# fulcrumgenomics/fgumi

Measured on AMD Instinct MI355X. Metric: simplex consensus throughput, input raw reads/s (depth-8 x 150bp), higher is better.
Workload: dtype f64

## Files before the change

### fgumi_amd/csrc/api.cpp

```cpp
#include <chrono>
#include <cstdio>
#include <stdexcept>
#include <cstring>
#include <mutex>
#include <map>
#include <mutex>
#include <string>
#include <thread>
#include "engine.h"
#include <gnu/libc-version.h>
#include <cmath>
#include "fastpath.h"
#include "host_common.h"
#include "simgen.h"
#include "canon_core.h"
#include "reject_core.h"
#include "aln_tags_core.h"

namespace fgx {
using canon::CANON_KIND_DUPLEX; using canon::CANON_KIND_CODEC; using canon::CANON_KIND_SIMPLEX;
uint32_t launch_canon_molecules(hipStream_t s, int kind, const canon::Params& P, const canon::CodecParams& PC, const uint8_t* d_blob,
                                const uint64_t* d_rec_off, const uint32_t* d_rec_len, const uint32_t* d_grp_first, const uint32_t* d_def, uint32_t nd,
                                const uint64_t* d_first, uint8_t* d_out, const uint64_t* d_out_off, uint32_t* d_out_len, int* d_status,
                                canon::Delta* d_delta, DevBuf& slabs, canon::RefRuns* d_runs, const rej::Params* PS);
// ... 1360 lines not shown
  out4[1] = out4[0] - s2_tile_bytes(mean_records);
  out4[2] = (uint32_t)sizeof(FullItem);
  out4[3] = S2_FLAG_DESC_BYTES;
}
void fgx_debug_last_packed_rows(const fgx_caller* c, uint64_t* out2) {
  if (!out2) return;
  out2[0] = out2[1] = 0;
  if (c && c->fast) { out2[0] = c->fast->fp.last_packed_clean; out2[1] = c->fast->fp.last_packed_general; }
}
void fgx_debug_last_full_results(const fgx_caller* c, uint64_t* out4) {
  if (!out4) return;
  for (int i = 0; i < 4; i++) out4[i] = (c && c->fast) ? c->fast->fp.last_full_results[i] : 0;
}
uint64_t fgx_debug_last_full_results_over(const fgx_caller* c) { return (c && c->fast) ? c->fast->fp.last_full_results[4] : 0; }
int fgx_debug_full_range_whole(uint32_t base, uint32_t items, uint32_t cap) { return full_range_whole(base, items, cap) ? 1 : 0; }
void fgx_debug_last_chain(const fgx_caller* c, uint32_t* out2) { if (out2) { out2[0] = (c && c->fast) ? c->fast->fp.last_launches : 0u; out2[1] = (c && c->fast) ? c->fast->fp.last_host_syncs : 0u; } }
uint32_t fgx_debug_last_routed(const fgx_caller* c) { return (c && c->fast) ? c->fast->fp.last_routed : 0u; }
int fgx_debug_last_direct(const fgx_caller* c) { return (c && c->fast) ? c->fast->fp.last_direct : 0; }
void fgx_set_general_only(fgx_caller* c, int on) { if (c) c->general_only = on != 0; }
void fgx_set_fast_lds_bytes(fgx_caller* c, uint32_t bytes) { if (c) { if (!c->fast) c->fast = new FastState(); c->fast->fp.lds_tile_bytes_large = bytes; } }

int fgx_call_columns(fgx_caller* c, const uint8_t* bases, const uint8_t* quals, uint32_t n_cols, uint32_t depth, uint8_t* out_base,
                     uint8_t* out_qual, uint32_t* out_depth, uint32_t* out_errors) {
  if (!c) return 1;
  c->err.clear();
  try {
    ColumnBatch& B = c->batch;
    B.clear();
    std::vector<uint8_t> rb, rq;
    for (uint32_t j0 = 0; j0 < n_cols; j0 += 4096) {
// ... 137 lines not shown
```

### fgumi_amd/csrc/fastpath.h

```cpp
#pragma once
#include <algorithm>
#include "engine.h"

#if defined(__HIPCC__)
#define FP_HD __host__ __device__ __forceinline__
#else
#define FP_HD inline
#endif

namespace fgx {

constexpr int FAST_RX_CAP = 48;

struct EndDesc {
  uint64_t col_off;
  uint64_t first_off;
  uint64_t kept_off;
  uint32_t cons_len;
  uint32_t rec_size;
  uint16_t mi_off, cb_off;
  uint8_t mi_len, cb_len, rx_len, type;
  uint8_t has_cb, has_rx, valid, meth;
  char rx[FAST_RX_CAP];
};
// ... 41 lines not shown
  return mean_need > floor16 ? std::min<uint32_t>((mean_need + 15u) & ~15u, 17408u) : floor16;
}
constexpr uint32_t FULL_ITEM_OBS = 0x80000000u;
constexpr uint32_t FULL_ITEM_CONT = 0x40000000u;

struct FullResult {
  uint32_t w0;
  uint32_t w1;
};
static_assert(sizeof(FullResult) == 8, "a result is one 8-byte store");
constexpr uint32_t FULL_RESULT_NONE = 0xFFu;
constexpr uint32_t FULL_RESULT_MAX_ITEMS = 64;
#ifndef FGX_FULL_RESULTS_DEFAULT
#define FGX_FULL_RESULTS_DEFAULT 1
#endif
constexpr int FULL_STATS_N = 5, FULL_STATS_STRIDE = 8;
FP_HD uint64_t full_range_word(uint32_t first, uint32_t items, bool whole) {
  return (uint64_t)first | ((uint64_t)(items < 0xFFFFu ? items : 0xFFFFu) << 32) | ((uint64_t)(whole ? 1u : 0u) << 48);
}
FP_HD bool full_range_whole(uint32_t base, uint32_t items, uint32_t cap) { return base < cap && items <= cap - base; }
FP_HD bool emit_pair_takes(uint32_t Lc1, uint32_t Lc2, uint32_t name_len, uint32_t rg_len, uint32_t mi_len, uint32_t cbl1, uint32_t cbl2,
                                                uint32_t rxl1, uint32_t rxl2, bool same_first, uint64_t dcol, uint64_t dout) {
  return Lc1 >= 8u && Lc1 <= 256u && Lc2 >= 8u && Lc2 <= 256u && name_len + 1u <= 32u && rg_len + 4u <= 32u && mi_len + 4u <= 32u &&
         cbl1 + 4u <= 32u && cbl2 + 4u <= 32u && rxl1 + 4u <= 32u && rxl2 + 4u <= 32u && rxl1 <= (uint32_t)FAST_RX_CAP && rxl2 <= (uint32_t)FAST_RX_CAP &&
         same_first && dcol < (1ull << 30) && dout - 1ull < (1ull << 30) - 1ull;
}
FP_HD bool full_results_family(bool packed, bool pair, bool whole, uint32_t items, bool pair_taken) {
  return packed && pair && whole && items <= FULL_RESULT_MAX_ITEMS && pair_taken;
}

struct SplitRec {
  uint32_t body_off;
  uint16_t seq_rel;
  uint16_t l_seq;
  uint16_t clip;
  uint16_t ov_off1, ov_off2, ov_cnt;
  uint8_t slot, mate_slot;
  uint8_t bits;
  uint8_t cb_len;
  uint16_t cb_rel, mi_rel;
  uint8_t mi_len, rx_len;
  uint16_t rx_rel;
  uint32_t _pad;
// ... 116 lines not shown
  const uint8_t* d_out; uint64_t out_len; uint64_t count;
  uint64_t stats[FGX_STATS_LEN];
  uint32_t n_deferred; const uint32_t* d_deferred;
  const uint64_t* d_out_off;
  const uint64_t* d_slot_size;
  uint32_t n_slots;
  double ms_kernels, ms_k_family, ms_k_emit; uint64_t cols_used; uint64_t full_items;
};

struct FastPath {
  DevBuf d_ends, d_sizes, d_offsets, d_code, d_qual, d_depth, d_err, d_misc, d_deferred, d_out, d_scan_tmp, d_strings;
  uint32_t lds_tile_bytes = 12288;
  uint32_t lds_tile_bytes_large = 65536;
  DevBuf d_retry, d_bound, d_colbase, d_statslots, d_full_items, d_full_count, d_obs, d_obs_all, d_retry2, d_retry_old;
  DevBuf d_full_res, d_full_flag;
  uint64_t last_full_results[FULL_STATS_N] = {0, 0, 0, 0, 0};
  DevBuf d_w2img;
  DevBuf d_famdesc;
  DevBuf d_fwimg;
  DevBuf d_split_rec, d_split_fam, d_split_out, d_route, d_s2img;
  DevBuf d_big;
  uint32_t last_big_families = 0;
  uint32_t last_deep_families = 0;
  DevBuf d_deep_sizes, d_deep_row0, d_deep_rows, d_deep_fams, d_deep_out, d_deep_out2;
  uint32_t last_wide_families = 0;
  DevBuf d_wide_scratch, d_wide_pass, d_wide_pass0, d_wide_depth;
  DevBuf d_mflag, d_mu, d_mt, d_mslot, d_mcontigs;
  const void* ref_runs = nullptr;
  uint32_t last_meth_device = 0;
  uint32_t last_meth_clipped = 0;
  uint32_t last_routed = 0;
// ... 29 lines not shown
```

### fgumi_amd/csrc/fastpath.hip

```cpp
#if !defined(FGX_WAVEMU)
#include <hipcub/hipcub.hpp>
#endif
#include "bamrec.h"
#include "canon_core.h"
#include "engine.h"
#include <cstdlib>
#include <memory>
#include <string>
#include <type_traits>
#include "fastpath.h"
#include "gate_core.h"
#include "packed_core.h"
#include "record_core.h"

#if defined(FGX_WAVEMU)
#define FGX_DYN_LDS(name) uint8_t* const name = wavemu::dyn_lds()
#define FGX_PIN(...) ((void)0)
#define FGX_UNDEF4(a, b, c, d) do { a = 0; b = 0; c = 0; d = 0; } while (0)
#define FGX_MEM_PIN() ((void)0)
#define FGX_CONST_AS
#else
#define FGX_DYN_LDS(name) extern __shared__ __align__(16) uint8_t name[]
#define FGX_PIN(...) asm volatile("" : __VA_ARGS__)
#define FGX_UNDEF4(a, b, c, d) asm volatile("" : "=v"(a), "=v"(b), "=v"(c), "=v"(d))
// ... 2587 lines not shown
enum MiscWord : uint32_t {
  MISC_STATS = 0,
  MISC_COLS_USED = 28,
  MISC_N_DEFERRED = 29,
  MISC_N_METH_CLIPPED = 30,
  MISC_N_RETRY = 31,
  MISC_N_RETRY_OLD = 32,
  MISC_N_ROUTE = 33,
  MISC_SMALL_RECS = 35,
  MISC_DIR_FLAGS = 36,
  MISC_N_BIG = 37,
  MISC_N_DEEP = 38,
  MISC_BUILD_FAMILIES = 40,
  MISC_N_SLOW = 44,
  MISC_FULL_RESULTS = 46,
  MISC_READ_BACK = 51,
  MISC_WORDS = 52
};
constexpr uint32_t MISC_SPLIT_WINDOW = MISC_N_BIG - MISC_N_RETRY + 1;
static_assert(FGX_STATS_LEN <= MISC_COLS_USED && MISC_BUILD_FAMILIES == 40 && MISC_BUILD_FAMILIES + (32 - FGX_STATS_LEN) <= MISC_N_SLOW,
              "k_reduce_stats writes words [0, FGX_STATS_LEN) and 40 .. of misc");
static_assert(MISC_N_METH_CLIPPED == MISC_N_DEFERRED + 1 && MISC_N_METH_CLIPPED < MISC_READ_BACK, "meth_clipped_counter: the word behind the deferred count");
static_assert(MISC_N_RETRY < MISC_N_ROUTE && MISC_N_ROUTE < MISC_N_BIG && MISC_SPLIT_WINDOW == 7 && MISC_N_SLOW < MISC_READ_BACK && MISC_READ_BACK <= MISC_WORDS, "misc layout");

inline bool env_not0(const char* e) { return !(e && e[0] == '0'); }
inline bool env_is1(const char* e) { return e && e[0] == '1'; }
inline int env_int(const char* e, int dflt) { return e ? atoi(e) : dflt; }
inline uint32_t env_in(const char* e, int lo, int hi, uint32_t dflt) { const int v = e ? atoi(e) : 0; return v >= lo && v <= hi ? (uint32_t)v : dflt; }

struct ProcessSwitches {
  const bool v2 = env_not0(fgx_knob("FGX_V2")), seg = env_not0(fgx_knob("FGX_SEG"));
  const bool seg2 = env_is1(fgx_knob("FGX_SEG2"));
  const bool early = env_not0(fgx_knob("FGX_S2_EARLY"));
  const int chunks = env_int(getenv("FGX_SPLIT_CHUNKS"), 0);
  const int nosum = env_int(fgx_knob("FGX_S2_NOSUM"), 1);
  const int packed = env_int(getenv("FGX_S2_PACKED"), 1);
  const bool clean_rows = env_not0(getenv("FGX_S2_CLEAN_ROWS"));
  const bool full_results = FGX_FULL_RESULTS_DEFAULT ? env_not0(getenv("FGX_FULL_RESULTS")) : env_is1(getenv("FGX_FULL_RESULTS"));
// ... 1 lines not shown
  const int pace = env_int(fgx_knob("FGX_S2_PACE"), 1);
  const uint32_t s2_bytes = env_in(fgx_knob("FGX_S2_BYTES"), 2048, 32768, 0) & ~15u, s2_wpb = env_in(fgx_knob("FGX_S2_WPB"), 1, 4, 0);
  const int s2_partner = env_int(fgx_knob("FGX_S2_PARTNER"), -1);
  const int s2_fixed = env_int(fgx_knob("FGX_S2_FIXED"), -1);
  const bool later_packed = env_not0(fgx_knob("FGX_S2_LATER_PACKED"));
  const bool verbose = env_is1(fgx_knob("FGX_S2_VERBOSE"));
  const uint32_t seg_wpb = env_in(fgx_knob("FGX_SEG_WPB"), 1, WAVES_PER_BLOCK, WAVES_PER_BLOCK), w2_wpb = env_in(fgx_knob("FGX_W2_WPB"), 1, WAVES_PER_BLOCK, FGX_W2_WPB_DEFAULT),
                 fw_wpb = env_in(fgx_knob("FGX_FW_WPB"), 1, WAVES_PER_BLOCK, WAVES_PER_BLOCK);
};
struct BatchSwitches {
  const char* const split_env = getenv("FGX_SPLIT");
  const bool split = env_not0(split_env);
  const int split_mode = env_int(split_env, 1);
  const bool direct = env_is1(getenv("FGX_DIRECT"));
  const bool deep = env_not0(getenv("FGX_DEEP"));
  const char* const deep_wide_env = getenv("FGX_DEEP_WIDE");
  const bool deep_wide = deep_wide_env && deep_wide_env[0] && deep_wide_env[0] != '0';
  const uint32_t seg_bytes = env_in(fgx_knob("FGX_SEG_BYTES"), 4096, 32768, 11776) & ~63u;
  const uint32_t wave_bytes = env_in(fgx_knob("FGX_WAVE_BYTES"), 1024, 22016, 0) & ~15u;
  const uint32_t lds_tile_large = env_in(fgx_knob("FGX_LDS_TILE_LARGE"), 16384, 163840, 0) & ~15u;
  const uint32_t split_fpw = env_in(fgx_knob("FGX_SPLIT_FPW"), 1, 32, 0);
};

#define FGX_LDS_ATTR(bytes, ...) lds_attr((const void*)__VA_ARGS__, bytes, #__VA_ARGS__)
void lds_attr(const void* kernel, int bytes, const char* name) {
  const hipError_t e = hipFuncSetAttribute(kernel, hipFuncAttributeMaxDynamicSharedMemorySize, bytes);
  if (e != hipSuccess) hip_check(e, (std::string("hipFuncSetAttribute(MaxDynamicSharedMemorySize) for ") + name + ": the device refused the dynamic LDS size").c_str());
}

struct Slice { uint32_t bytes, wpb; int build; };
// ... 200 lines not shown
    fp.d_retry.reserve((size_t)n_grp * 4);
    P.retry = fp.d_retry.as<uint32_t>(); P.n_retry = cnt(MISC_N_RETRY);
    const uint64_t full_total = col_cap / fp.pool_div + (uint64_t)N_LISTS * fp.pool_slack;
    full_cap = (uint32_t)std::min<uint64_t>(full_total / N_LISTS, 0x7FFFFFFFull);
    fp.d_full_items.reserve((size_t)full_cap * N_LISTS * sizeof(FullItem));
    fp.d_full_count.reserve((size_t)N_LISTS * 4);
    hip_check(hipMemsetAsync(fp.d_full_count.p, 0, (size_t)N_LISTS * 4, s), "memset");
    P.full_items = fp.d_full_items.as<FullItem>(); P.full_count = fp.d_full_count.as<uint32_t>(); P.full_cap = full_cap;
    full_results = ps.full_results && FGX_EMIT_PAIR != 0 && !duplex && !codec && !direct && !meth_dev && (uint64_t)full_cap * N_LISTS <= 0xFFFFFFFFull;
    fp.d_full_res.reserve(FULL_STATS_BYTES + (full_results ? (size_t)full_cap * N_LISTS * sizeof(FullResult) : 0));
    hip_check(hipMemsetAsync(fp.d_full_res.p, 0, FULL_STATS_BYTES, s), "memset");
    P.full_stats = fp.d_full_res.as<unsigned long long>();
    if (full_results) {
      fp.d_full_flag.reserve((size_t)n_grp + 16);
      hip_check(hipMemsetAsync(fp.d_full_flag.p, 0, (size_t)n_grp, s), "memset");
      P.full_results = 1; P.full_flag = fp.d_full_flag.as<uint8_t>();
    }
    P.lds_wave_bytes = sw.wave_bytes ? sw.wave_bytes : duplex ? fp.lds_wave_bytes_duplex : codec ? fp.lds_wave_bytes_codec : fp.lds_wave_bytes;
    P.lds_tile_bytes = fp.lds_tile_bytes_large;
    if (!fp.lds_attr_set) {
      FGX_LDS_ATTR(WAVES_PER_BLOCK * 22016, k_family_wave<0>);
      FGX_LDS_ATTR(WAVES_PER_BLOCK * 22016, k_family_wave<1>);
      FGX_LDS_ATTR(WAVES_PER_BLOCK * 22016, k_family_wave<2>);
      FGX_LDS_ATTR(WAVES_PER_BLOCK * 22016, k_family_wave<1, 1>);
      FGX_LDS_ATTR(WAVES_PER_BLOCK * 22016, k_family_wave<1, 0, 1>);
      FGX_LDS_ATTR(WAVES_PER_BLOCK * 22016, k_family_wave<2, 0, 1>);
      fp.lds_attr_set = true;
    }
    fp.d_retry2.reserve((size_t)n_grp * 4);
    lists[0] = fp.d_retry.as<uint32_t>(); lists[1] = fp.d_retry2.as<uint32_t>();
    if (!duplex && !codec && !direct) { fp.d_big.reserve((size_t)n_grp * 4); P.big = fp.d_big.as<uint32_t>(); P.n_big = cnt(MISC_N_BIG); }
// ... 65 lines not shown
      const bool pair_build = B.packed && (ci == 0 || ps.later_packed);
      if (ci == 0) {
        for (uint32_t k = 0; k < n_chunks; k++) {
          const uint32_t ga = k * chunk_fam, gb = (uint32_t)std::min<uint64_t>((uint64_t)ga + chunk_fam, n_grp);
          if (ga >= gb) break;
          hip_check(hipStreamWaitEvent(s, fp.ev_chunk[k], 0), "wait");
          if (S.build) launch_split_cols<160, 80>(S, pair_build, PS, ga, gb - ga); else launch_split_cols<0, 0>(S, pair_build, PS, ga, gb - ga);
          hip_check(hipEventRecord(fp.ev_cols[k], s), "event");
          hip_check(hipStreamWaitEvent(fp.s2, fp.ev_cols[k], 0), "wait");
          FastParams PF = P;
          PF.group_list = nullptr; PF.g0 = ga;
          FGX_LAUNCH(k_split_finish, dim3((gb - ga + 255) / 256), dim3(256), 0, fp.s2, PF, gb - ga);
          if (paced && k + 2 < n_chunks) launch_parse(k + 2, dir_scan_bytes);
        }
      } else {
        if (S.build) launch_split_cols<160, 80>(S, pair_build, PS, 0u, n_cur); else launch_split_cols<0, 0>(S, pair_build, PS, 0u, n_cur);
        FastParams PF = P;
        PF.group_list = cur_list; PF.g0 = 0;
        FGX_LAUNCH(k_split_finish, dim3((n_cur + 255) / 256), dim3(256), 0, s, PF, n_cur);
      }
      unsigned long long h_cnt[MISC_SPLIT_WINDOW] = {};
      hip_check(hipMemcpyAsync(h_cnt, misc + MISC_N_RETRY, sizeof(h_cnt), hipMemcpyDeviceToHost, s), "D2H");
      split_counts_seen = true;
      sync();
      const uint32_t n_next = PS.retry ? (uint32_t)h_cnt[0] : 0u;
      h_route_seen = (uint32_t)h_cnt[MISC_N_ROUTE - MISC_N_RETRY]; h_big_seen = (uint32_t)h_cnt[MISC_N_BIG - MISC_N_RETRY];
      if (ci == 0) fp.last_first_stage_retries = n_next;
      next_list(n_next);
    }
    hip_check(hipEventRecord(fp.ev_fin, fp.s2), "event");
// ... 470 lines not shown
```

### fgumi_amd/csrc/record_writers.inc

```

__device__ __forceinline__ uint8_t int_tag_byte(uint32_t j, char a, char b, uint32_t v) {
  return j == 0 ? (uint8_t)a : j == 1 ? (uint8_t)b : j == 2 ? (uint8_t)(v <= 127 ? 'c' : v <= 255 ? 'C' : 'S') : j == 3 ? (uint8_t)v : (uint8_t)(v >> 8);
}

#ifndef FGX_EMIT_FLAT
#define FGX_EMIT_FLAT 1
#endif
struct EmitCtx {
  uint8_t* q; const uint8_t* first; const uint8_t* code; const uint8_t* cq; const uint16_t* cd; const uint16_t* ce;
  uint32_t Lc, name_len, mi_len, mi_off, flag, rec_size;
};

__device__ __forceinline__ uint32_t gld32u(const uint8_t* p) { uint32_t v; __builtin_memcpy(&v, p, 4); return v; }
__device__ __forceinline__ uint2 gld64u(const uint8_t* p) { uint2 v; __builtin_memcpy(&v, p, 8); return v; }
__device__ __forceinline__ void gst32u(uint8_t* p, uint32_t v) { __builtin_memcpy(p, &v, 4); }
__device__ __forceinline__ void gst16u(uint8_t* p, uint32_t v) { const uint16_t w = (uint16_t)v; __builtin_memcpy(p, &w, 2); }

struct FieldWriterNested {
  uint8_t* q; uint32_t lane;
  static __device__ __forceinline__ uint8_t head3(uint32_t i, char t0, char t1) { return i == 0 ? (uint8_t)t0 : i == 1 ? (uint8_t)t1 : (uint8_t)'Z'; }
  static __device__ __forceinline__ uint8_t head8(uint32_t i, char t0, char t1, uint32_t L) {
    return i == 0 ? (uint8_t)t0 : i == 1 ? (uint8_t)t1 : i == 2 ? (uint8_t)'B' : i == 3 ? (uint8_t)'s' : (uint8_t)(L >> (8 * ((i - 4) & 3)));
  }
  template <class F> __device__ __forceinline__ void small(uint32_t n, F f) { if (lane < n) q[lane] = f(lane); q += n; }
// ... 275 lines not shown
#endif
}

constexpr uint32_t EMIT_PATCH_BYTES = 64u * (8u + 8u + 16u + 16u);
#ifndef FGX_EMIT_PAIR
#define FGX_EMIT_PAIR 1
#endif
typedef unsigned short em_u16x2 __attribute__((ext_vector_type(2)));
__device__ __forceinline__ uint32_t em_pkmax(uint32_t a, uint32_t b) { em_u16x2 x, y; __builtin_memcpy(&x, &a, 4); __builtin_memcpy(&y, &b, 4); x = __builtin_elementwise_max(x, y); uint32_t r; __builtin_memcpy(&r, &x, 4); return r; }
__device__ __forceinline__ uint32_t em_pkmin(uint32_t a, uint32_t b) { em_u16x2 x, y; __builtin_memcpy(&x, &a, 4); __builtin_memcpy(&y, &b, 4); x = __builtin_elementwise_min(x, y); uint32_t r; __builtin_memcpy(&r, &x, 4); return r; }
__device__ __forceinline__ uint32_t em_sum2(uint32_t pair, uint32_t acc) { em_u16x2 x; const em_u16x2 one = {1, 1}; __builtin_memcpy(&x, &pair, 4); return __builtin_amdgcn_udot2(x, one, acc, false); }
#define FGX_HALF_REDUCE(v, idn, OP) do { \
    v = OP(v, wave_dpp<0xB1, 0xF>(idn, v)); v = OP(v, wave_dpp<0x4E, 0xF>(idn, v)); v = OP(v, wave_dpp<0x141, 0xF>(idn, v)); v = OP(v, wave_dpp<0x140, 0xF>(idn, v)); \
    v = OP(v, wave_dpp<0x142, 0xA>(idn, v)); } while (0)
__device__ __forceinline__ bool emit_pair(const EmitParams& P, const EndDesc* D , uint64_t oo1, uint64_t oo2, uint32_t lane,
                                          uint8_t* const patch, const uint32_t fr_first, const uint32_t fr_cnt) {
  typedef uint32_t u32x4 __attribute__((ext_vector_type(4)));
  const EndDesc& D1 = D[1];
  const EndDesc& D2 = D[2];
  const uint32_t Lc1 = uni(D1.cons_len), Lc2 = uni(D2.cons_len);
  const uint32_t mi_len = uni(D1.mi_len), mi_off = uni(D1.mi_off);
  const uint64_t first_off = uniform_u64(D1.first_off);
  const uint64_t col1 = uniform_u64(D1.col_off), col2 = uniform_u64(D2.col_off);
  const bool hcb1 = uni(D1.has_cb) != 0, hcb2 = uni(D2.has_cb) != 0, hrx1 = uni(D1.has_rx) != 0, hrx2 = uni(D2.has_rx) != 0;
  const uint32_t cbl1 = hcb1 ? uni(D1.cb_len) : 0u, cbl2 = hcb2 ? uni(D2.cb_len) : 0u, rxl1 = hrx1 ? uni(D1.rx_len) : 0u, rxl2 = hrx2 ? uni(D2.rx_len) : 0u;
  const uint32_t name_len = P.prefix_len + 1u + mi_len, rg_len = P.rg_len;
  const bool ok = emit_pair_takes(Lc1, Lc2, name_len, rg_len, mi_len, cbl1, cbl2, rxl1, rxl2,
                                  uniform_u64(D2.first_off) == first_off && uni(D2.mi_len) == mi_len && uni(D2.mi_off) == mi_off, col2 - col1, oo2 - oo1);
  if (!ok) return false;
  const uint32_t l = lane & 31u;
  const bool hb = lane >= 32u;
// ... 3 lines not shown
  const uint32_t d_type = hb ? ty2 : ty1, rec_size = hb ? rs2 : rs1;
  const bool hcb = hb ? hcb2 : hcb1, hrx = hb ? hrx2 : hrx1;
  const uint32_t cb_len = hb ? cbl2 : cbl1, rx_len = hb ? rxl2 : rxl1;
  const uint32_t n0 = 8u * l;
  const bool pay = n0 < Lc;
  const uint32_t c0 = min(n0, Lc - 8u);
  const uint32_t cs = min(n0, ((Lc + 1u) & ~1u) - 8u);
  const uint8_t* const code = P.col_code + col1;
  const uint8_t* const cq = P.col_qual + col1;
  const uint8_t* const cdb = (const uint8_t*)(P.col_depth + col1);
  const uint8_t* const ceb = (const uint8_t*)(P.col_err + col1);
  uint2 cw = gld64u(code + (dcol + cs));
  uint2 qw = gld64u(cq + (dcol + c0));
  u32x4 dv, ev;
  __builtin_memcpy(&dv, cdb + 2u * (dcol + c0), 16);
  __builtin_memcpy(&ev, ceb + 2u * (dcol + c0), 16);
  FullResult fr;
  fr.w0 = FULL_RESULT_NONE << 16; fr.w1 = 0u;
  if (fr_cnt != 0u && lane < fr_cnt) { const uint2 v = *(const uint2*)(P.full_res + ((size_t)fr_first + lane)); fr.w0 = v.x; fr.w1 = v.y; }
  const uint8_t* const first = P.blob + first_off;
  const uint32_t j3 = l >= 3u ? l - 3u : 0u;
  const uint32_t ni = l > P.prefix_len ? l - P.prefix_len - 1u : 0u;
  const uint8_t pfx = (uint8_t)P.prefix[l < P.prefix_len ? l : 0u];
  const uint8_t nmb = first[mi_off + (ni < mi_len ? ni : mi_len)];
  const uint8_t rgb = (uint8_t)P.rg[j3 < rg_len ? j3 : 0u];
  const uint8_t mib = first[mi_off + (j3 < mi_len ? j3 : mi_len)];
  uint8_t cbb = 0;
  if (hcb1 || hcb2) {
    const uint64_t k1 = hcb1 ? uniform_u64(D1.kept_off) + uni(D1.cb_off) : first_off, k2 = hcb2 ? uniform_u64(D2.kept_off) + uni(D2.cb_off) : first_off;
    const uint8_t* const fk = P.blob + (hb ? k2 : k1);
    cbb = fk[j3 < cb_len ? j3 : 0u];
// ... 156 lines not shown
  const uint64_t oo = P.out_off[s0 + (lane < ns ? lane : 0u)];
#if FGX_EMIT_PAIR
  const uint32_t fr_flag = (P.full_flag && !P.fam_list) ? (uint32_t)P.full_flag[fam] : 0u;
#endif
  if (lane < 6 * ns) ((u32x4*)&sD[wv][0])[lane] = piece;
  wave_sync();
  const bool v0 = uni(sD[wv][0].valid) != 0, v1 = ns > 1 && uni(sD[wv][1].valid) != 0, v2 = ns > 2 && uni(sD[wv][2].valid) != 0;
  auto off_of = [&](int k) -> uint64_t {
    return ((uint64_t)(uint32_t)__builtin_amdgcn_readlane((int)(uint32_t)(oo >> 32), k) << 32) | (uint32_t)__builtin_amdgcn_readlane((int)(uint32_t)oo, k);
  };
  if (v0) { EmitLoads R0; emit_load(P, sD[wv][0], off_of(0), lane, R0); emit_store(P, sD[wv][0], lane, R0); }
#if FGX_EMIT_PAIR
  {
    const uint64_t fr_word = uniform_u64(sD[wv][0].col_off);
    const uint32_t fr_cnt = uni(fr_flag) ? (uint32_t)(fr_word >> 32) & 0xFFFFu : 0u;
    if (!v0 && v1 && v2 && emit_pair(P, &sD[wv][0], off_of(1), off_of(2), lane, &sPatch[wv][0], (uint32_t)fr_word, fr_cnt <= FULL_RESULT_MAX_ITEMS ? fr_cnt : 0u)) return;
  }
#endif
  EmitLoads R1, R2;
  if (v1) emit_load(P, sD[wv][1], off_of(1), lane, R1);
  if (v2) emit_load(P, sD[wv][2], off_of(2), lane, R2);
  if (v1) emit_store(P, sD[wv][1], lane, R1);
  if (v2) emit_store(P, sD[wv][2], lane, R2);
}

constexpr uint32_t DUP_SLOTS = 2;

__device__ __forceinline__ bool small_tags(uint32_t name_len, uint32_t mi_len, uint32_t cb_len, uint32_t rg_len, uint32_t rx_len) {
  return name_len + 1 <= 64 && mi_len + 4 <= 64 && cb_len + 4 <= 64 && rg_len + 4 <= 64 && rx_len + 4 <= 64;
}
__device__ __forceinline__ bool fast_ok(const DuplexDesc& D, uint32_t prefix_len, uint32_t rg_len) {
// ... 494 lines not shown
```

### fgumi_amd/csrc/simplex_split.inc

```

#ifndef FGX_S2_OCC
#define FGX_S2_OCC 6
#endif
#ifndef FGX_S2_OCC_PACKED
#define FGX_S2_OCC_PACKED 7
#endif
#ifndef FGX_S2_PAIRS
#define FGX_S2_PAIRS 256
#endif

#ifndef FGX_S2_F32
#define FGX_S2_F32 1
#endif
#ifndef FGX_S2_FMASEL
#define FGX_S2_FMASEL 1
#endif
#ifndef FGX_S2_NOSUM
#define FGX_S2_NOSUM 1
#endif
#ifndef FGX_S2_PREGATE
#define FGX_S2_PREGATE 1
#endif
struct S2Lds {
  GateTables g;
// ... 1065 lines not shown
          const uint32_t sh = bsel & 16u, dv = dcol << sh;
          acc_max = s2_pkmax(acc_max, dv); acc_min = s2_pkmin(acc_min, dv | (0xFFFF0000u >> sh)); acc_sum += dv;
        }
      } else if (incol && !cold && resolved) {
        uint8_t ob, oq;
        if (n1 < P.min_reads) { ob = 15; oq = 0; }
        else if (q_call < P.min_cons_bq) { ob = 15; oq = FGX_MIN_PHRED; }
        else { ob = (uint8_t)code_call; oq = (uint8_t)q_call; }
        fam_code[oc] = ob; fam_qual[oc] = oq; fam_err[oc] = 0;
      }
    }
    }
  };
  uint32_t ires_early = 0;
  bool ires_asked = false;
  auto run_cols_packed = [&](const uint32_t cnt_a, const uint32_t cnt_b, const uint32_t m, const bool last_run) -> bool {
    const uint32_t nsafe = P.s2_nsafe;
    const uint32_t ga = cnt_a ? (len_a + 7u) >> 3 : 0u, gb = cnt_b ? (len_b + 7u) >> 3 : 0u;
    const bool dbg = (P.s2_packed & 2u) != 0;
    if (!(P.s2_packed && m >= nsafe && m <= S2_PACKED_MAX_ROWS && P.min_reads <= nsafe && min_bq <= 128u && ((QS & 7u) | (SS & 3u)) == 0u && ga + gb <= 64u &&
          S0 + n * SS < 65536u && lc_a + lc_b < 65536u)) {
      if (dbg && lane == 0) atomicAdd(&g_s2_dbg[42], 1u);
      return false;
    }
    if (dbg && lane == 0) atomicAdd(&g_s2_dbg[0], 1u);
    const bool in_b = lane >= ga, inl = lane < ga + gb;
    const uint32_t k = inl ? (in_b ? lane - ga : lane) : 0u;
    const bool lrev = (in_b ? rev_b : rev_a) != 0;
    const uint32_t lenE = in_b ? len_b : len_a, cntE = in_b ? cnt_b : cnt_a;
    const uint32_t rowE = in_b ? m_a : 0u;
    const uint32_t qaddr0 = s2_mul24(rowE, QS) + 8u * k, saddr0 = S0 + s2_mul24(rowE, SS) + 4u * k;
// ... 30 lines not shown
    const uint32_t T = uni((uint32_t)__popcll(pb0) + 2u * (uint32_t)__popcll(pb1) + 4u * (uint32_t)__popcll(pb2) + 8u * (uint32_t)__popcll(pb3));
    const uint32_t oc0 = (in_b ? offB : offA) + (uint32_t)c_lo;
    const uint32_t list = (P.lds_wave_bytes - 8u * T) & ~7u;
    if (T && (8u * T + 8u > P.lds_wave_bytes || ibase + icnt * (uint32_t)sizeof(FullItem) > list)) {
      if (dbg && lane == 0) atomicAdd(&g_s2_dbg[3], 1u);
      gone = true; return true;
    }
    (void)last_run;
    (void)full2; (void)lo_s;
    if (hi_s > lo_s) {
      const Planes PL = planes();
      const uint2 cv = make_uint2(code2[0], code2[1]), qv = make_uint2(qual2[0], qual2[1]);
      const u32x4 dv = {dep4[0], dep4[1], dep4[2], dep4[3]}, zv = {0u, 0u, 0u, 0u};
      const uint32_t o1 = oc0, o2 = 2u * oc0;
      __builtin_memcpy(PL.code + o1, &cv, 8); __builtin_memcpy(PL.qual + o1, &qv, 8);
      __builtin_memcpy((uint8_t*)PL.depth + o2, &dv, 16); __builtin_memcpy((uint8_t*)PL.err + o2, &zv, 16);
    }
    PH(12)
    if (T) {
      uint32_t pre = mbcnt64(pb0) + 2u * mbcnt64(pb1) + 4u * mbcnt64(pb2) + 8u * mbcnt64(pb3);
      while (fm) {
        const uint32_t bi = (uint32_t)__builtin_ctz(fm), slot = (bi >> 3) | (bi & 4u);
        fm &= fm - 1u;
        const uint32_t pos = lrev ? 7u - slot : slot;
        const uint2 d = make_uint2((qaddr0 + pos) | ((saddr0 + (pos >> 1)) << 16), (oc0 + slot) | (((~pos & 1u) << 2) << 16) | ((lrev ? 1u : 0u) << 20));
        *(uint2*)(W + list + 8u * pre) = d;
        pre++;
      }
      PH(11)
      wave_sync();
      const auto& K6 = KA::of(P);
// ... 37 lines not shown
          if (dbg && lane == 0) atomicAdd(&g_s2_dbg[3], 1u);
          gone = true; return true;
        }
        if (need) {
          uint8_t* const it = W + ibase + s2_mul24(icnt + per_cold * (uint32_t)__popcll(needm & below0), (uint32_t)sizeof(FullItem));
          if (on) *(uint16_t*)(it + (j >> 4) * (uint32_t)sizeof(FullItem) + 8 + 2 * (j & 15u)) = (uint16_t)ob16;
          if (j == 0u) { *(uint64_t*)it = col_base + oc_l; *(uint32_t*)(it + 40) = g + 1u; *(uint32_t*)(it + 44) = FULL_ITEM_OBS | m; }
          if (j == 16u && per_cold > 1u) { *(uint32_t*)(it + sizeof(FullItem) + 40) = g + 1u; *(uint32_t*)(it + sizeof(FullItem) + 44) = FULL_ITEM_CONT; }
        } else if (col_on && j == r1) {
          const uint32_t nobs = one ? 1u : 2u;
          uint32_t ob, oq;
          if (nobs < P.min_reads) { ob = 15; oq = 0; }
          else if (tq < P.min_cons_bq) { ob = 15; oq = FGX_MIN_PHRED; }
          else { ob = c1; oq = tq; }
          PL.code[oc_l] = (uint8_t)ob; PL.qual[oc_l] = (uint8_t)oq;
          *(uint16_t*)((uint8_t*)PL.depth + 2u * oc_l) = (uint16_t)nobs; *(uint16_t*)((uint8_t*)PL.err + 2u * oc_l) = (uint16_t)0;
        }
        icnt = uni(icnt + n_need);
      }
    }
    PH(13)
    if (dbg && lane == 0) { atomicAdd(&g_s2_dbg[1], 1u); atomicAdd(&g_s2_dbg[2], T); }
    return true;
  };
  if constexpr (COLS == 1) {
    leave(__any(dirty_v != 0u) ? 0x81u : 0xC1u, (ne << 8) | (type_a << 16) | (fk_a << 24), fk_b | (surv_a << 8) | (surv_b << 16) | (n << 24), lc_a | (lc_b << 16), rej, ov_agree, ov_dis);
    if (lane == 0) ((uint32_t*)&KA::of(P).split_out[g])[6] = ov_corr;
  }
  {
    const bool multi_a = ne >= 1u && surv_a >= 2u, multi_b = ne == 2u && surv_b >= 2u;
    if constexpr (DIRECT != 0) {
      if (ne >= 1u && surv_a == 1u) single_end_direct(mem_a, RA, false);
      if (ne == 2u && surv_b == 1u) single_end_direct(mem_b, RB, true);
    } else {
      if (ne >= 1u && surv_a == 1u) single_end(mem_a, lc_a, offA);
      if (ne == 2u && surv_b == 1u) single_end(mem_b, lc_b, offB);
    }
    const bool both = multi_a && multi_b && m_a == m_b;
    const uint32_t nruns = both ? 1u : (multi_a ? 1u : 0u) + (multi_b ? 1u : 0u);
    if constexpr (COLS == 1) {
      if (nruns != 0u) {
        const bool run_a = both || multi_a;
        if (!run_cols_packed(run_a ? lc_a : 0u, (both || !run_a) ? lc_b : 0u, run_a ? m_a : m_b, nruns == 1u)) gone = true;
      }
      if (nruns == 2u && !gone) { if (!run_cols_packed(0u, lc_b, m_b, true)) gone = true; }
    } else {
#pragma unroll 1
      for (uint32_t ri = 0; ri < nruns && !gone; ri++) {
        const bool first_is_a = both || multi_a;
        const bool run_a = ri == 0 && first_is_a, run_b = both || !run_a;
        const uint32_t rc_a = run_a ? lc_a : 0u, rc_b = run_b ? lc_b : 0u, rc_m = run_a ? m_a : m_b;
        run_cols(rc_a, rc_b, rc_m);
      }
    }
    if (gone) { if (gone_far) to_route(); else to_retry(); return; }
  }
  PH(6)
  S2_ABLATE_AFTER(6, icnt + rej + ov_bases + ov_corr)

  uint32_t ires = 0;
// ... 53 lines not shown
      const uint32_t rem = icnt - done;
      const uint32_t fit = base < full_cap ? (rem < full_cap - base ? rem : full_cap - base) : 0u;
      const uint4* src = (const uint4*)(W + ibase) + 3 * done;
      uint4* dst = (uint4*)(full_items + ((size_t)l * full_cap + base));
      for (uint32_t c = lane; c < 3 * fit; c += 64) dst[c] = src[c];
      done += fit;
      if (done == icnt) break;
      if (++tries >= N_LISTS) { overflow = true; break; }
      l = (l + 1) & (N_LISTS - 1);
      uint32_t b2 = 0;
      if (lane == 0) b2 = atomicAdd(&KA::of(P).full_count[l], icnt - done);
      base = uni(b2);
    }
    }
    if (overflow) {
      leave(3u, 0, 0, 0, 0, 0, 0);
      if (DIRECT) dir_tables(0, 0, 0);
      if (lane == 0) { uint32_t kk = atomicAdd(KA::of(P).n_deferred, 1u); KA::of(P).deferred[kk] = g; }
      return;
    }
  }
  if constexpr (COLS == 1 && DIRECT == 0) { if (lane == 0) KA::of(P).ends[slot0].col_off = full_range_word(fr_first, icnt, fr_whole); }
  (void)fr_first; (void)fr_whole;
  PH(8)
}

template <int QS_T, int SS_T, int DIRECT, int COLS>
__global__ __launch_bounds__(256, COLS == 1 ? FGX_S2_OCC_PACKED : FGX_S2_OCC) void k_split_cols(FastParams P, uint32_t n_grp_total) {
  FGX_DYN_LDS(dyn);
  typedef typename S2SharedOf<COLS>::type S2Shared;
  __shared__ __align__(16) S2Shared sL;
  typedef s2_u32x4 u32x4;
  const uint32_t lane = threadIdx.x & 63, wv = threadIdx.x >> 6;
  const uint32_t gi_raw = blockIdx.x * (blockDim.x >> 6) + wv;
  bool bail = gi_raw >= n_grp_total;
  const uint32_t gi = bail ? 0u : gi_raw;
  const uint32_t g = P.group_list ? P.group_list[gi] : P.g0 + gi;
// ... 20 lines not shown
    else if (threadIdx.x == 24u) tiny_w = w[(offsetof(S2Lds, g) + offsetof(GateTables, cap)) / 4];
  } else {
#pragma unroll
    for (int u = 0; u < 6; u++) { const uint32_t ii = threadIdx.x + u * blockDim.x; im[u] = img_src[ii < IMG_V ? ii : 0u]; }
  }
  uint8_t* W = dyn + (size_t)wv * P.lds_wave_bytes;
  const uint32_t my_list = blockIdx.x & (N_LISTS - 1);
  s2_cols_family<QS_T, SS_T, DIRECT, COLS, false>(P, g, bail, tiny_w, im, W, sL, lane, my_list);
}

__global__ __launch_bounds__(256) void k_split_finish(FastParams P, uint32_t count) {
  typedef uint32_t u32x4 __attribute__((ext_vector_type(4)));
  const uint32_t gi = blockIdx.x * blockDim.x + threadIdx.x;
  const uint32_t lane = threadIdx.x & 63;
  uint32_t c_total = 0, c_cons = 0, c_insuf = 0, c_zero = 0, c_orphan = 0, c_agree = 0, c_dis = 0, c_corr = 0, c_packed = 0, c_classic = 0, c_clean = 0;
  uint32_t c_apply = 0, c_cut = 0, c_over = 0;
  if (gi < count) {
    const uint32_t g = P.group_list ? P.group_list[gi] : P.g0 + gi;
    const SplitOut O = P.split_out[g];
    const uint32_t slot0 = 3 * g;
    const uint32_t o_status = O.status & 0x3Fu;
    const bool padded = (O.status & 0x80u) != 0;
    const bool clean = (O.status & 0x40u) != 0;
    if (o_status == 2) { c_total = O.n; c_insuf = O.n; }
    const bool direct = P.out != nullptr;
    if (o_status != 0 && !direct) {
      EndDesc* D = &P.ends[slot0];
      D[0].valid = 0; D[1].valid = 0; D[2].valid = 0;
      P.rec_sizes[slot0] = 0; P.rec_sizes[slot0 + 1] = 0; P.rec_sizes[slot0 + 2] = 0;
    }
    if (o_status == 1) {
// ... 105 lines not shown
        const u32x4 p1 = {(uint32_t)kept_off, (uint32_t)(kept_off >> 32), Lc, size};
        const u32x4 p2 = {(uint32_t)R0.mi_rel | ((uint32_t)RK.cb_rel << 16), mi0_len | (cbl << 8) | (rx_ulen << 16) | (e_type << 24),
                          (hcb ? 1u : 0u) | ((rx_cnt ? 1u : 0u) << 8) | (1u << 16), rxw[0]};
        const u32x4 p3 = {rxw[1], rxw[2], rxw[3], rxw[4]}, p4 = {rxw[5], rxw[6], rxw[7], rxw[8]}, p5 = {rxw[9], rxw[10], rxw[11], 0u};
        u32x4* dst = (u32x4*)&P.ends[slot0 + e_type];
        dst[0] = p0; dst[1] = p1; dst[2] = p2; dst[3] = p3; dst[4] = p4; dst[5] = p5;
        P.rec_sizes[slot0 + e_type] = (uint64_t)size + 4;
        fr_cbl[k & 1u] = hcb ? cbl : 0u; fr_rxl[k & 1u] = rx_cnt ? rx_ulen : 0u;
        if (k == 0) fr_size0 = size;
      }
      if (fr_pair) {
        const uint32_t items = (uint32_t)(fr_word >> 32) & 0xFFFFu;
        const bool whole = ((fr_word >> 48) & 1u) != 0;
        const bool taken = emit_pair_takes(O.lc_a, O.lc_b, P.prefix_len + 1u + R0.mi_len, P.rg_len, R0.mi_len, fr_cbl[0], fr_cbl[1], fr_rxl[0], fr_rxl[1], true,
                                           (uint64_t)(s2_padded_b(O.lc_a) - S2_PAD_FRONT), (uint64_t)fr_size0 + 4ull);
        if (full_results_family(true, true, whole, items, taken)) { c_apply = 1u; P.full_flag[g] = 1; }
        else if (taken) { if (!whole) c_cut = 1u; else c_over = 1u; }
      }
    }
  }
  const uint32_t t_cons = wave_sum(c_cons), t_total = wave_sum(c_total), t_insuf = wave_sum(c_insuf), t_zero = wave_sum(c_zero), t_orphan = wave_sum(c_orphan);
  const uint32_t t_agree = wave_sum(c_agree), t_dis = wave_sum(c_dis), t_corr = wave_sum(c_corr);
  const uint32_t t_packed = wave_sum(c_packed), t_classic = wave_sum(c_classic);
  const uint32_t t_clean = wave_sum(c_clean);
  if (lane == 0) {
    unsigned long long* st = P.stats + (size_t)((blockIdx.x * 4 + (threadIdx.x >> 6)) & (STAT_SLOTS - 1)) * 32;
    if (t_total) atomicAdd(&st[0], (unsigned long long)t_total);
    if (t_cons) atomicAdd(&st[1], (unsigned long long)t_cons);
    const uint32_t filt = t_insuf + t_zero + t_orphan;
    if (filt) atomicAdd(&st[2], (unsigned long long)filt);
    if (t_insuf) atomicAdd(&st[3 + FGX_REJ_INSUFFICIENT_READS], (unsigned long long)t_insuf);
    if (t_zero) atomicAdd(&st[3 + FGX_REJ_ZERO_LENGTH_AFTER_TRIMMING], (unsigned long long)t_zero);
    if (t_orphan) atomicAdd(&st[3 + FGX_REJ_ORPHAN_CONSENSUS], (unsigned long long)t_orphan);
    if (t_agree + t_dis) atomicAdd(&st[24], (unsigned long long)(t_agree + t_dis));
    if (t_agree) atomicAdd(&st[25], (unsigned long long)t_agree);
    if (t_dis) atomicAdd(&st[26], (unsigned long long)t_dis);
    if (t_corr) atomicAdd(&st[27], (unsigned long long)t_corr);
    if (t_packed) atomicAdd(&st[28], (unsigned long long)t_packed);
    if (t_classic) atomicAdd(&st[29], (unsigned long long)t_classic);
    if (t_clean) atomicAdd(&st[30], (unsigned long long)t_clean);
    if (t_packed - t_clean) atomicAdd(&st[31], (unsigned long long)(t_packed - t_clean));
  }
  if (P.full_results) {
    const uint32_t t_apply = wave_sum(c_apply), t_cut = wave_sum(c_cut), t_over = wave_sum(c_over);
    if (lane == 0) {
      unsigned long long* fs = P.full_stats + (size_t)((blockIdx.x * 4 + (threadIdx.x >> 6)) & (STAT_SLOTS - 1)) * FULL_STATS_STRIDE;
      if (t_apply) atomicAdd(&fs[2], (unsigned long long)t_apply);
      if (t_cut) atomicAdd(&fs[3], (unsigned long long)t_cut);
      if (t_over) atomicAdd(&fs[4], (unsigned long long)t_over);
    }
  }
}
```

Measured before the change: 3.182 billion.

## Skip zero error-plane stores and loads for packed simplex pair families

Packed single-run simplex pair families that qualify for full results no longer write the all-zero error plane. Instead a NO_ERR bit is set in the range word and in the per-family flag, and the emit kernel substitutes zeros rather than loading the error columns. Families that cannot take the path still get their zeros, either as a deferred store or as a fallback fill in the finalize kernel. The change also adds a cross-stream event wait before the first split chunk, extra full-result counters and debug hooks, which adds control-flow complexity and a possible serialization point.

```diff
diff --git a/fgumi_amd/csrc/api.cpp b/fgumi_amd/csrc/api.cpp
--- a/fgumi_amd/csrc/api.cpp
+++ b/fgumi_amd/csrc/api.cpp
@@ -1398,6 +1398,19 @@
 }
 uint64_t fgx_debug_last_full_results_over(const fgx_caller* c) { return (c && c->fast) ? c->fast->fp.last_full_results[4] : 0; }
 int fgx_debug_full_range_whole(uint32_t base, uint32_t items, uint32_t cap) { return full_range_whole(base, items, cap) ? 1 : 0; }
+void fgx_debug_last_err_plane(const fgx_caller* c, uint64_t* out2) {
+  if (!out2) return;
+  for (int i = 0; i < 2; i++) out2[i] = (c && c->fast) ? c->fast->fp.last_full_results[5 + i] : 0;
+}
+int fgx_debug_err_plane_rule(int enabled, int pair, int one_run, uint32_t base, uint32_t items, uint32_t cap, const uint32_t* f) {
+  if (!f) return 0;
+  const bool whole = full_range_whole(base, items, cap);
+  const bool taken_cols = emit_pair_takes(f[0], f[1], f[2], f[3], f[4], f[5], f[6], f[7], f[8], true, f[9], EMIT_PAIR_DOUT_ANY);
+  const bool taken_fin = emit_pair_takes(f[0], f[1], f[2], f[3], f[4], f[5], f[6], f[7], f[8], true, f[9], f[10]);
+  const bool skipped = err_plane_skipped(enabled != 0, pair != 0, one_run != 0, whole, items, taken_cols);
+  const bool family = full_results_family(pair != 0, pair != 0, whole, items < 0xFFFFu ? items : 0xFFFFu, taken_fin);
+  return (skipped ? 1 : 0) | (family ? 2 : 0);
+}
 void fgx_debug_last_chain(const fgx_caller* c, uint32_t* out2) { if (out2) { out2[0] = (c && c->fast) ? c->fast->fp.last_launches : 0u; out2[1] = (c && c->fast) ? c->fast->fp.last_host_syncs : 0u; } }
 uint32_t fgx_debug_last_routed(const fgx_caller* c) { return (c && c->fast) ? c->fast->fp.last_routed : 0u; }
 int fgx_debug_last_direct(const fgx_caller* c) { return (c && c->fast) ? c->fast->fp.last_direct : 0; }
diff --git a/fgumi_amd/csrc/fastpath.h b/fgumi_amd/csrc/fastpath.h
--- a/fgumi_amd/csrc/fastpath.h
+++ b/fgumi_amd/csrc/fastpath.h
@@ -79,10 +79,12 @@
 #ifndef FGX_FULL_RESULTS_DEFAULT
 #define FGX_FULL_RESULTS_DEFAULT 1
 #endif
-constexpr int FULL_STATS_N = 5, FULL_STATS_STRIDE = 8;
-FP_HD uint64_t full_range_word(uint32_t first, uint32_t items, bool whole) {
-  return (uint64_t)first | ((uint64_t)(items < 0xFFFFu ? items : 0xFFFFu) << 32) | ((uint64_t)(whole ? 1u : 0u) << 48);
-}
+constexpr int FULL_STATS_N = 7, FULL_STATS_STRIDE = 8;
+constexpr uint64_t FULL_RANGE_NO_ERR = 1ull << 49;
+FP_HD uint64_t full_range_word(uint32_t first, uint32_t items, bool whole, bool no_err = false) {
+  return (uint64_t)first | ((uint64_t)(items < 0xFFFFu ? items : 0xFFFFu) << 32) | ((uint64_t)(whole ? 1u : 0u) << 48) | (no_err ? FULL_RANGE_NO_ERR : 0ull);
+}
+constexpr uint8_t FULL_FLAG_APPLY = 1, FULL_FLAG_NO_ERR = 2;
 FP_HD bool full_range_whole(uint32_t base, uint32_t items, uint32_t cap) { return base < cap && items <= cap - base; }
 FP_HD bool emit_pair_takes(uint32_t Lc1, uint32_t Lc2, uint32_t name_len, uint32_t rg_len, uint32_t mi_len, uint32_t cbl1, uint32_t cbl2,
                                                 uint32_t rxl1, uint32_t rxl2, bool same_first, uint64_t dcol, uint64_t dout) {
@@ -92,6 +94,10 @@
 }
 FP_HD bool full_results_family(bool packed, bool pair, bool whole, uint32_t items, bool pair_taken) {
   return packed && pair && whole && items <= FULL_RESULT_MAX_ITEMS && pair_taken;
+}
+constexpr uint64_t EMIT_PAIR_DOUT_ANY = 1ull;
+FP_HD bool err_plane_skipped(bool enabled, bool packed_pair, bool one_run, bool whole, uint32_t items, bool pair_taken) {
+  return enabled && one_run && full_results_family(packed_pair, packed_pair, whole, items, pair_taken);
 }
 
 struct SplitRec {
@@ -238,7 +244,7 @@
   uint32_t lds_tile_bytes_large = 65536;
   DevBuf d_retry, d_bound, d_colbase, d_statslots, d_full_items, d_full_count, d_obs, d_obs_all, d_retry2, d_retry_old;
   DevBuf d_full_res, d_full_flag;
-  uint64_t last_full_results[FULL_STATS_N] = {0, 0, 0, 0, 0};
+  uint64_t last_full_results[FULL_STATS_N] = {0, 0, 0, 0, 0, 0, 0};
   DevBuf d_w2img;
   DevBuf d_famdesc;
   DevBuf d_fwimg;
diff --git a/fgumi_amd/csrc/fastpath.hip b/fgumi_amd/csrc/fastpath.hip
--- a/fgumi_amd/csrc/fastpath.hip
+++ b/fgumi_amd/csrc/fastpath.hip
@@ -2625,14 +2625,15 @@
   MISC_BUILD_FAMILIES = 40,
   MISC_N_SLOW = 44,
   MISC_FULL_RESULTS = 46,
-  MISC_READ_BACK = 51,
-  MISC_WORDS = 52
+  MISC_READ_BACK = 53,
+  MISC_WORDS = 54
 };
 constexpr uint32_t MISC_SPLIT_WINDOW = MISC_N_BIG - MISC_N_RETRY + 1;
 static_assert(FGX_STATS_LEN <= MISC_COLS_USED && MISC_BUILD_FAMILIES == 40 && MISC_BUILD_FAMILIES + (32 - FGX_STATS_LEN) <= MISC_N_SLOW,
               "k_reduce_stats writes words [0, FGX_STATS_LEN) and 40 .. of misc");
 static_assert(MISC_N_METH_CLIPPED == MISC_N_DEFERRED + 1 && MISC_N_METH_CLIPPED < MISC_READ_BACK, "meth_clipped_counter: the word behind the deferred count");
 static_assert(MISC_N_RETRY < MISC_N_ROUTE && MISC_N_ROUTE < MISC_N_BIG && MISC_SPLIT_WINDOW == 7 && MISC_N_SLOW < MISC_READ_BACK && MISC_READ_BACK <= MISC_WORDS, "misc layout");
+static_assert(MISC_FULL_RESULTS + FULL_STATS_N <= MISC_READ_BACK && FULL_STATS_N <= FULL_STATS_STRIDE && 32 + FULL_STATS_N <= 64, "k_reduce_stats: a thread per counter of the result array");
 
 inline bool env_not0(const char* e) { return !(e && e[0] == '0'); }
 inline bool env_is1(const char* e) { return e && e[0] == '1'; }
@@ -2664,6 +2665,7 @@
   const int split_mode = env_int(split_env, 1);
   const bool direct = env_is1(getenv("FGX_DIRECT"));
   const bool deep = env_not0(getenv("FGX_DEEP"));
+  const bool err_skip = env_not0(getenv("FGX_ERR_SKIP"));
   const char* const deep_wide_env = getenv("FGX_DEEP_WIDE");
   const bool deep_wide = deep_wide_env && deep_wide_env[0] && deep_wide_env[0] != '0';
   const uint32_t seg_bytes = env_in(fgx_knob("FGX_SEG_BYTES"), 4096, 32768, 11776) & ~63u;
@@ -2894,7 +2896,7 @@
     if (full_results) {
       fp.d_full_flag.reserve((size_t)n_grp + 16);
       hip_check(hipMemsetAsync(fp.d_full_flag.p, 0, (size_t)n_grp, s), "memset");
-      P.full_results = 1; P.full_flag = fp.d_full_flag.as<uint8_t>();
+      P.full_results = sw.err_skip ? 3u : 1u; P.full_flag = fp.d_full_flag.as<uint8_t>();
     }
     P.lds_wave_bytes = sw.wave_bytes ? sw.wave_bytes : duplex ? fp.lds_wave_bytes_duplex : codec ? fp.lds_wave_bytes_codec : fp.lds_wave_bytes;
     P.lds_tile_bytes = fp.lds_tile_bytes_large;
@@ -2990,6 +2992,7 @@
           if (paced && k + 2 < n_chunks) launch_parse(k + 2, dir_scan_bytes);
         }
       } else {
+        if (ci == 1) { hip_check(hipEventRecord(fp.ev_fin, fp.s2), "event"); hip_check(hipStreamWaitEvent(s, fp.ev_fin, 0), "wait"); }
         if (S.build) launch_split_cols<160, 80>(S, pair_build, PS, 0u, n_cur); else launch_split_cols<0, 0>(S, pair_build, PS, 0u, n_cur);
         FastParams PF = P;
         PF.group_list = cur_list; PF.g0 = 0;
diff --git a/fgumi_amd/csrc/record_writers.inc b/fgumi_amd/csrc/record_writers.inc
--- a/fgumi_amd/csrc/record_writers.inc
+++ b/fgumi_amd/csrc/record_writers.inc
@@ -313,7 +313,7 @@
     v = OP(v, wave_dpp<0xB1, 0xF>(idn, v)); v = OP(v, wave_dpp<0x4E, 0xF>(idn, v)); v = OP(v, wave_dpp<0x141, 0xF>(idn, v)); v = OP(v, wave_dpp<0x140, 0xF>(idn, v)); \
     v = OP(v, wave_dpp<0x142, 0xA>(idn, v)); } while (0)
 __device__ __forceinline__ bool emit_pair(const EmitParams& P, const EndDesc* D , uint64_t oo1, uint64_t oo2, uint32_t lane,
-                                          uint8_t* const patch, const uint32_t fr_first, const uint32_t fr_cnt) {
+                                          uint8_t* const patch, const uint32_t fr_first, const uint32_t fr_cnt, const bool err_zero) {
   typedef uint32_t u32x4 __attribute__((ext_vector_type(4)));
   const EndDesc& D1 = D[1];
   const EndDesc& D2 = D[2];
@@ -347,7 +347,8 @@
   uint2 qw = gld64u(cq + (dcol + c0));
   u32x4 dv, ev;
   __builtin_memcpy(&dv, cdb + 2u * (dcol + c0), 16);
-  __builtin_memcpy(&ev, ceb + 2u * (dcol + c0), 16);
+  ev = (u32x4){0u, 0u, 0u, 0u};
+  if (!err_zero) __builtin_memcpy(&ev, ceb + 2u * (dcol + c0), 16);
   FullResult fr;
   fr.w0 = FULL_RESULT_NONE << 16; fr.w1 = 0u;
   if (fr_cnt != 0u && lane < fr_cnt) { const uint2 v = *(const uint2*)(P.full_res + ((size_t)fr_first + lane)); fr.w0 = v.x; fr.w1 = v.y; }
@@ -534,7 +535,8 @@
   {
     const uint64_t fr_word = uniform_u64(sD[wv][0].col_off);
     const uint32_t fr_cnt = uni(fr_flag) ? (uint32_t)(fr_word >> 32) & 0xFFFFu : 0u;
-    if (!v0 && v1 && v2 && emit_pair(P, &sD[wv][0], off_of(1), off_of(2), lane, &sPatch[wv][0], (uint32_t)fr_word, fr_cnt <= FULL_RESULT_MAX_ITEMS ? fr_cnt : 0u)) return;
+    if (!v0 && v1 && v2 && emit_pair(P, &sD[wv][0], off_of(1), off_of(2), lane, &sPatch[wv][0], (uint32_t)fr_word, fr_cnt <= FULL_RESULT_MAX_ITEMS ? fr_cnt : 0u,
+                                     (uni(fr_flag) & FULL_FLAG_NO_ERR) != 0u)) return;
   }
 #endif
   EmitLoads R1, R2;
diff --git a/fgumi_amd/csrc/simplex_split.inc b/fgumi_amd/csrc/simplex_split.inc
--- a/fgumi_amd/csrc/simplex_split.inc
+++ b/fgumi_amd/csrc/simplex_split.inc
@@ -1103,7 +1103,15 @@
   };
   uint32_t ires_early = 0;
   bool ires_asked = false;
-  auto run_cols_packed = [&](const uint32_t cnt_a, const uint32_t cnt_b, const uint32_t m, const bool last_run) -> bool {
+  bool err_skip_ok = false;
+  uint32_t err_o2 = ~0u;
+  auto err_zero_store = [&]() {
+    if constexpr (COLS == 1) {
+      uint8_t* const fam_err8 = (uint8_t*)(KA::of(P).col_err + col_base);
+      if (err_o2 != ~0u) { const u32x4 zv = {0u, 0u, 0u, 0u}; __builtin_memcpy(fam_err8 + err_o2, &zv, 16); err_o2 = ~0u; }
+    }
+  };
+  auto run_cols_packed = [&](const uint32_t cnt_a, const uint32_t cnt_b, const uint32_t m, const bool last_run, const bool hold_err) -> bool {
     const uint32_t nsafe = P.s2_nsafe;
     const uint32_t ga = cnt_a ? (len_a + 7u) >> 3 : 0u, gb = cnt_b ? (len_b + 7u) >> 3 : 0u;
     const bool dbg = (P.s2_packed & 2u) != 0;
@@ -1164,7 +1172,8 @@
       const u32x4 dv = {dep4[0], dep4[1], dep4[2], dep4[3]}, zv = {0u, 0u, 0u, 0u};
       const uint32_t o1 = oc0, o2 = 2u * oc0;
       __builtin_memcpy(PL.code + o1, &cv, 8); __builtin_memcpy(PL.qual + o1, &qv, 8);
-      __builtin_memcpy((uint8_t*)PL.depth + o2, &dv, 16); __builtin_memcpy((uint8_t*)PL.err + o2, &zv, 16);
+      __builtin_memcpy((uint8_t*)PL.depth + o2, &dv, 16);
+      if (hold_err) err_o2 = o2; else __builtin_memcpy((uint8_t*)PL.err + o2, &zv, 16);
     }
     PH(12)
     if (T) {
@@ -1232,7 +1241,7 @@
           else if (tq < P.min_cons_bq) { ob = 15; oq = FGX_MIN_PHRED; }
           else { ob = c1; oq = tq; }
           PL.code[oc_l] = (uint8_t)ob; PL.qual[oc_l] = (uint8_t)oq;
-          *(uint16_t*)((uint8_t*)PL.depth + 2u * oc_l) = (uint16_t)nobs; *(uint16_t*)((uint8_t*)PL.err + 2u * oc_l) = (uint16_t)0;
+          *(uint16_t*)((uint8_t*)PL.depth + 2u * oc_l) = (uint16_t)nobs;
         }
         icnt = uni(icnt + n_need);
       }
@@ -1256,12 +1265,24 @@
     }
     const bool both = multi_a && multi_b && m_a == m_b;
     const uint32_t nruns = both ? 1u : (multi_a ? 1u : 0u) + (multi_b ? 1u : 0u);
+    if constexpr (COLS == 1 && DIRECT == 0) {
+      const FastParams& K5 = P;
+      const uint32_t fa = uni(fk_a), fb = uni(fk_b);
+      const uint32_t mi0 = rlane(mi_len, 0), rxl = rx_all ? rx_ulen : 0u, bits_a = rlane(bits, fa), bits_b = rlane(bits, fb), cb_a = rlane(cb_len, fa), cb_b = rlane(cb_len, fb);
+      uint32_t tags4;
+      __builtin_memcpy(&tags4, &K5.tag0, 4);
+      const bool cell = ((tags4 >> 16) & 0xFFu) != 0u;
+      const uint32_t cbl_a = (cell && (bits_a & 8u)) ? cb_a : 0u, cbl_b = (cell && (bits_b & 8u)) ? cb_b : 0u;
+      const bool taken = emit_pair_takes(lc_a, lc_b, K5.prefix_len + 1u + mi0, K5.rg_len, mi0, cbl_a, cbl_b, rxl, rxl, true, (uint64_t)(s2_padded_b(lc_a) - S2_PAD_FRONT), EMIT_PAIR_DOUT_ANY);
+      err_skip_ok = uni(err_plane_skipped((K5.full_results & 2u) != 0u, ne == 2u && type_a == 1u, both, true, 0u, taken) ? 1u : 0u) != 0u;
+    }
     if constexpr (COLS == 1) {
       if (nruns != 0u) {
         const bool run_a = both || multi_a;
-        if (!run_cols_packed(run_a ? lc_a : 0u, (both || !run_a) ? lc_b : 0u, run_a ? m_a : m_b, nruns == 1u)) gone = true;
-      }
-      if (nruns == 2u && !gone) { if (!run_cols_packed(0u, lc_b, m_b, true)) gone = true; }
+        if (!run_cols_packed(run_a ? lc_a : 0u, (both || !run_a) ? lc_b : 0u, run_a ? m_a : m_b, nruns == 1u, true)) gone = true;
+      }
+      if (!both || gone) err_zero_store();
+      if (nruns == 2u && !gone) { if (!run_cols_packed(0u, lc_b, m_b, true, false)) gone = true; }
     } else {
 #pragma unroll 1
       for (uint32_t ri = 0; ri < nruns && !gone; ri++) {
@@ -1345,13 +1366,18 @@
     }
     }
     if (overflow) {
+      err_zero_store();
       leave(3u, 0, 0, 0, 0, 0, 0);
       if (DIRECT) dir_tables(0, 0, 0);
       if (lane == 0) { uint32_t kk = atomicAdd(KA::of(P).n_deferred, 1u); KA::of(P).deferred[kk] = g; }
       return;
     }
   }
-  if constexpr (COLS == 1 && DIRECT == 0) { if (lane == 0) KA::of(P).ends[slot0].col_off = full_range_word(fr_first, icnt, fr_whole); }
+  if constexpr (COLS == 1 && DIRECT == 0) {
+    const bool no_err = err_skip_ok && err_plane_skipped(true, true, true, fr_whole, icnt, true);
+    if (!no_err) err_zero_store();
+    if (lane == 0) KA::of(P).ends[slot0].col_off = full_range_word(fr_first, icnt, fr_whole, no_err);
+  }
   (void)fr_first; (void)fr_whole;
   PH(8)
 }
@@ -1402,7 +1428,7 @@
   const uint32_t gi = blockIdx.x * blockDim.x + threadIdx.x;
   const uint32_t lane = threadIdx.x & 63;
   uint32_t c_total = 0, c_cons = 0, c_insuf = 0, c_zero = 0, c_orphan = 0, c_agree = 0, c_dis = 0, c_corr = 0, c_packed = 0, c_classic = 0, c_clean = 0;
-  uint32_t c_apply = 0, c_cut = 0, c_over = 0;
+  uint32_t c_apply = 0, c_cut = 0, c_over = 0, c_noerr = 0, c_fill = 0;
   if (gi < count) {
     const uint32_t g = P.group_list ? P.group_list[gi] : P.g0 + gi;
     const SplitOut O = P.split_out[g];
@@ -1538,8 +1564,16 @@
         const bool whole = ((fr_word >> 48) & 1u) != 0;
         const bool taken = emit_pair_takes(O.lc_a, O.lc_b, P.prefix_len + 1u + R0.mi_len, P.rg_len, R0.mi_len, fr_cbl[0], fr_cbl[1], fr_rxl[0], fr_rxl[1], true,
                                            (uint64_t)(s2_padded_b(O.lc_a) - S2_PAD_FRONT), (uint64_t)fr_size0 + 4ull);
-        if (full_results_family(true, true, whole, items, taken)) { c_apply = 1u; P.full_flag[g] = 1; }
+        const bool no_err = (fr_word & FULL_RANGE_NO_ERR) != 0;
+        const bool applied = full_results_family(true, true, whole, items, taken);
+        if (applied) { c_apply = 1u; c_noerr = no_err ? 1u : 0u; P.full_flag[g] = no_err ? (uint8_t)(FULL_FLAG_APPLY | FULL_FLAG_NO_ERR) : FULL_FLAG_APPLY; }
         else if (taken) { if (!whole) c_cut = 1u; else c_over = 1u; }
+        if (no_err && !applied) {
+          c_fill = 1u;
+          uint16_t* const e = P.col_err + col_base;
+          for (uint32_t i = 0; i < (uint32_t)O.lc_a; i++) e[S2_PAD_FRONT + i] = 0;
+          for (uint32_t i = 0; i < (uint32_t)O.lc_b; i++) e[s2_padded_b(O.lc_a) + i] = 0;
+        }
       }
     }
   }
@@ -1567,11 +1601,14 @@
   }
   if (P.full_results) {
     const uint32_t t_apply = wave_sum(c_apply), t_cut = wave_sum(c_cut), t_over = wave_sum(c_over);
+    const uint32_t t_noerr = wave_sum(c_noerr), t_fill = wave_sum(c_fill);
     if (lane == 0) {
       unsigned long long* fs = P.full_stats + (size_t)((blockIdx.x * 4 + (threadIdx.x >> 6)) & (STAT_SLOTS - 1)) * FULL_STATS_STRIDE;
       if (t_apply) atomicAdd(&fs[2], (unsigned long long)t_apply);
       if (t_cut) atomicAdd(&fs[3], (unsigned long long)t_cut);
       if (t_over) atomicAdd(&fs[4], (unsigned long long)t_over);
+      if (t_noerr) atomicAdd(&fs[5], (unsigned long long)t_noerr);
+      if (t_fill) atomicAdd(&fs[6], (unsigned long long)t_fill);
     }
   }
 }
```

Result: no change. 3.156 billion (-0.8%).
